# iracigt/ceres-raytracer

Measured on AMD Instinct MI355X. Metric: Mrays/sec (primary+shadow) on dragon.obj 1920x1080; 1/2/4/8-GPU scaling, higher is better.
Workload: dtype f32; 1 GPU; dragon_1080: dragon.obj 1920x1080 primary+shadow, 16 copies of the config view per step; views=config, W=1920, H=1080, row_block=1080, parallelism=one GPU, whole frames, float_framebuffer=True, streams=8

## Files before the change

### ceres-raytracer_amd/__init__.py

```python
import ctypes
import os
import sys

import numpy as np

_PKG = os.path.dirname(os.path.abspath(__file__))
LIB_PATH = os.environ.get("CERES_LIB") or os.path.join(_PKG, "libceres_hip.so")
CLI_PATH = os.path.join(_PKG, "render")

if _PKG not in sys.path:
    sys.path.insert(0, _PKG)
import configs

MODE_FULL, MODE_PRIMARY = 0, 1
MODE_ROBUST = 0x10
MODE_QBVH4 = 0x20
MODE_FMA = 0x40
ARITH_EXACT, ARITH_FMA = 0, 1


def cfg_mode(cfg, arith=ARITH_EXACT):
    return ((MODE_PRIMARY if cfg["mode"] == "primary" else MODE_FULL) | (MODE_ROBUST if cfg.get("robust") else 0)
            | (MODE_FMA if arith else 0))
SCENE_STATS = 1
# ... 5 lines not shown
    "ceres_device_free", "ceres_camera_basis", "ceres_obj_load_f64", "ceres_proc_mesh_f64", "ceres_rotate_triangles_f64",
    "ceres_bvh_build_f64", "ceres_camera_basis_f64", "ceres_orbit_cameras_f64", "ceres_scene_create_f64",
    "ceres_render_f64", "ceres_render_records_f64", "ceres_obj_load_f64_arith", "ceres_proc_mesh_f64_arith",
    "ceres_rotate_triangles_f64_arith", "ceres_bvh_build_f64_arith", "ceres_camera_basis_f64_arith",
    "ceres_orbit_cameras_f64_arith",
    "ceres_free", "ceres_scene_create", "ceres_scene_create_device", "ceres_scene_destroy", "ceres_scene_info", "ceres_scene_shadow_stacks", "ceres_render_f32",
    "ceres_render_device", "ceres_render_batch_device", "ceres_render_multi_f32", "ceres_device_count", "ceres_assemble_rgb8_packed", "ceres_render_records", "ceres_tiling_local_rows",
    "ceres_scene_set_timing", "ceres_scene_read_timing", "ceres_scene_wave_log", "ceres_fetch_counters",
    "ceres_cpu_scene_create", "ceres_cpu_scene_destroy", "ceres_render_cpu_f32", "ceres_cpu_scene_create_f64",
    "ceres_render_cpu_f64",
    "ceres_orbit_cameras", "ceres_assemble_rgb8",
    "ceres_kernel_names", "ceres_last_error", "ceres_version",
    "ceres_obj_load_arith", "ceres_proc_mesh_arith", "ceres_rotate_triangles_arith", "ceres_bvh_build_arith",
    "ceres_camera_basis_arith", "ceres_orbit_cameras_arith", "ceres_content_hash",
    "ceres_bvh_build_gpu_arith", "ceres_bvh_build_device_arith", "ceres_obj_load_gpu_arith",
    "ceres_obj_parse_device_arith", "ceres_rotate_triangles_device_arith",
)


class CeresError(RuntimeError):
    pass


class _Stats(ctypes.Structure):
    _fields_ = [("rays", ctypes.c_uint64), ("hits", ctypes.c_uint64), ("primary_rays", ctypes.c_uint64),
                ("shadow_rays", ctypes.c_uint64), ("node_pairs", ctypes.c_uint64), ("tri_tests", ctypes.c_uint64),
                ("ms", ctypes.c_double)]


class Tiling(ctypes.Structure):
    _fields_ = [("row_block", ctypes.c_uint32), ("rank", ctypes.c_uint32), ("world", ctypes.c_uint32),
# ... 112 lines not shown
    L.ceres_render_cpu_f64.argtypes = [_vp, _dp, _dp, ctypes.c_int, _dp, ctypes.POINTER(ctypes.c_uint8), _sz, _sz,
                                       ctypes.POINTER(_Stats), ctypes.c_int]
    L.ceres_content_hash.argtypes = [_vp, _sz]
    L.ceres_content_hash.restype = ctypes.c_uint64
    L.ceres_obj_load_arith.argtypes = L.ceres_obj_load.argtypes + [ctypes.c_int]
    L.ceres_proc_mesh_arith.argtypes = L.ceres_proc_mesh.argtypes + [ctypes.c_int]
    L.ceres_rotate_triangles_arith.argtypes = L.ceres_rotate_triangles.argtypes + [ctypes.c_int]
    L.ceres_bvh_build_arith.argtypes = L.ceres_bvh_build.argtypes + [ctypes.c_int]
    L.ceres_camera_basis_arith.argtypes = L.ceres_camera_basis.argtypes + [ctypes.c_int]
    L.ceres_orbit_cameras_arith.argtypes = L.ceres_orbit_cameras.argtypes + [ctypes.c_int]
    L.ceres_bvh_build_gpu_arith.argtypes = L.ceres_bvh_build_gpu.argtypes + [ctypes.c_int]
    L.ceres_bvh_build_device_arith.argtypes = L.ceres_bvh_build_device.argtypes + [ctypes.c_int]
    L.ceres_obj_load_gpu_arith.argtypes = L.ceres_obj_load_gpu.argtypes + [ctypes.c_int]
    L.ceres_obj_parse_device_arith.argtypes = L.ceres_obj_parse_device.argtypes + [ctypes.c_int]
    L.ceres_rotate_triangles_device_arith.argtypes = L.ceres_rotate_triangles_device.argtypes + [ctypes.c_int]
    _lib = L
    return L


def _check(rc):
    if rc != 0:
        raise CeresError(f"ceres error {rc}: {lib().ceres_last_error().decode()}")


def _p(a, t):
    return None if a is None else a.ctypes.data_as(ctypes.POINTER(t))


def _take(ptr, count, dtype):
    if count == 0:
# ... 127 lines not shown
    return Bvh(_take(nodes, m.value * 8, np.uint32).reshape(-1, 8), _take(prim, len(mesh), np.uint64))


def build_bvh_gpu(mesh, device=0, arith=ARITH_EXACT):
    nodes, prim, m = _u32p(), _u64p(), _sz()
    _check(lib().ceres_bvh_build_gpu_arith(_p(mesh.tri, ctypes.c_float), len(mesh), ctypes.byref(nodes),
                                           ctypes.byref(m), ctypes.byref(prim), int(device), int(arith)))
    return Bvh(_take(nodes, m.value * 8, np.uint32).reshape(-1, 8), _take(prim, len(mesh), np.uint64))


def build_bvh_device(d_tri48, n_tri, d_nodes32, d_prim32, stream=0, arith=ARITH_EXACT):
    m = _sz()
    _check(lib().ceres_bvh_build_device_arith(d_tri48, n_tri, d_nodes32, d_prim32, ctypes.byref(m), stream or None,
                                              int(arith)))
    return m.value


class CpuScene:

    def __init__(self, mesh, bvh):
        L = lib()
        self.f64 = mesh.f64
        if self.f64:
            self._h = L.ceres_cpu_scene_create_f64(_p(mesh.tri, ctypes.c_double), len(mesh), _p(mesh.norm, ctypes.c_double),
                                                   bvh.nodes.ctypes.data_as(_vp), bvh.nodes.shape[0],
                                                   _p(bvh.prim, ctypes.c_uint64))
        else:
            self._h = L.ceres_cpu_scene_create(_p(mesh.tri, ctypes.c_float), len(mesh), _p(mesh.norm, ctypes.c_float),
                                               bvh.nodes.ctypes.data_as(_vp), bvh.nodes.shape[0],
                                               _p(bvh.prim, ctypes.c_uint64))
# ... 299 lines not shown
```

### ceres-raytracer_amd/csrc/ceres_types.hpp

```cpp
#pragma once
#include <cstddef>
#include <cstdint>
#include <vector>

namespace ceres {

struct Tri48 {
    float p0[3], e1[3], e2[3], n[3];
};
static_assert(sizeof(Tri48) == 48, "Tri48");

struct RefNode {
    float bounds[6];
    uint32_t primitive_count;
    uint32_t first_child_or_primitive;
};
static_assert(sizeof(RefNode) == 32, "RefNode");

struct alignas(16) SiblingPair {
    float lb[6];
    float rb[6];
    uint32_t lcount, lfirst;
    uint32_t rcount, rfirst;
};
// ... 92 lines not shown
    uint32_t bands;
    uint32_t band_magic;
    uint32_t row_blocks_per_frame;
    uint32_t stack_entries;
    uint32_t root_leaf_count, root_leaf_first;
    float root_box[6];
    uint32_t root_box_ok;
    uint32_t cull;
    uint32_t shadow_stack_entries;
    uint32_t steal_first;
    uint32_t packets;
    uint32_t tiles_x;
    uint32_t lds_entries;
    uint32_t tile_packed;
    const uint32_t* tile_order;
    const SiblingPair* pairs;
    const Node4* nodes4;
    const QNode4* qnodes4;
    const Tri48* tris;
    const uint32_t* orig;
    const float* norms;
    float* pixels;
    uint8_t* rgb8;
    Shard* shards;
    int32_t* rec_prim;
    float* rec_tuv;
    int8_t* rec_shadow;
    unsigned long long* wave_log;
};
static_assert(sizeof(KParams) <= 4096, "KParams must fit the 4 KB kernel-argument limit");
// ... 27 lines not shown
```

### ceres-raytracer_amd/csrc/render_hip.hip

```cpp
#include <hip/hip_runtime.h>

#include <algorithm>
#include <chrono>
#include <cfloat>
#include <cmath>
#include <cstdint>
#include <cstdlib>
#include <cstring>
#include <new>
#include <string>
#include <type_traits>
#include <vector>

#include "ceres_render.h"
#include "ceres_types.hpp"
#include "host_common.hpp"
#include "pow24.hpp"

#pragma clang fp contract(off)

#ifndef CERES_COUNTING
#define CERES_COUNTING 0
#endif
#ifndef CERES_TILES_PER_WAVE
#define CERES_TILES_PER_WAVE 4
#endif
#ifndef CERES_TPW_BY_SIZE
#define CERES_TPW_BY_SIZE 1
#endif
#ifndef CERES_FRAME_MAJOR_PIXELS
#define CERES_FRAME_MAJOR_PIXELS (1u << 20)
#endif
#ifndef CERES_SPLIT_UNIFORM
#define CERES_SPLIT_UNIFORM 1
#endif
// ... 32 lines not shown
#endif
#ifndef CERES_RCP_UNIFORM
#define CERES_RCP_UNIFORM 2
#endif
#ifndef CERES_RCP_IFTHEN
#define CERES_RCP_IFTHEN 1
#endif
#ifndef CERES_PK_PACKET
#define CERES_PK_PACKET 1
#endif
#ifndef CERES_LOAD_ALWAYS
#define CERES_LOAD_ALWAYS 1
#endif
#ifndef CERES_CULL
#define CERES_CULL 1
#endif
#ifndef CERES_TRI_SELECT
#define CERES_TRI_SELECT 1
#endif

namespace ceres {

char* error_buffer() {
    static thread_local char buf[kErrorBufferSize] = "";
    return buf;
}

namespace dev {

constexpr int kBlock = 256;
// ... 239 lines not shown
        case 0: fn(std::integral_constant<int, 0>{}); break;
        case 1: fn(std::integral_constant<int, 1>{}); break;
        case 2: fn(std::integral_constant<int, 2>{}); break;
        case 3: fn(std::integral_constant<int, 3>{}); break;
        case 4: fn(std::integral_constant<int, 4>{}); break;
        case 5: fn(std::integral_constant<int, 5>{}); break;
        case 6: fn(std::integral_constant<int, 6>{}); break;
        default: fn(std::integral_constant<int, 7>{}); break;
    }
    return true;
}

template <bool kAnyHit, bool kStats, int kS = kBlock, typename StkT = uint32_t*, bool kRobust = false, int kOct = -1,
          bool kG = false>
__device__ __forceinline__ bool trace(const KParams& P, F3 o, F3 d, StkT stk, Hit& best,
                                      uint32_t& n_pairs, uint32_t& n_tests, bool& overflow) {
    const float tmin = 0.0f;
    float tmax = FLT_MAX;
    bool have = false;
    constexpr bool kU = CERES_RCP_UNIFORM == 1 || (CERES_RCP_UNIFORM == 2 && kOct == -2);
    if (P.root_leaf_count) {
        if (kStats) n_tests += P.root_leaf_count;
        for (uint32_t k = P.root_leaf_first; k < P.root_leaf_first + P.root_leaf_count; ++k) {
            float t, u, v;
            CERES_COUNT_V(kFTriV, 48);
            if (tri_test<kG, kU>(load_tri(P.tris + k), o, d, tmin, tmax, t, u, v)) {
                best = {k, t, u, v}; have = true;
                if (kAnyHit) return true;
                tmax = t;
            }
        }
        return have;
    }
    const Slab<kRobust> sl = make_slab<kRobust>(o, d);
    if constexpr (!kRobust && kOct == -1 && (CERES_OCTANT_SLAB & 1)) {
        bool r = false;
        if (with_uniform_octant(sl, [&](auto k) {
                r = trace<kAnyHit, kStats, kS, StkT, kRobust, decltype(k)::value, kG>(P, o, d, stk, best, n_pairs, n_tests, overflow);
            }))
            return r;
    }
    if (P.root_box_ok) {
        float e, x;
        slab_box<kRobust, kOct>(sl, P.root_box[0], P.root_box[1], P.root_box[2], P.root_box[3], P.root_box[4],
                          P.root_box[5], tmin, tmax, e, x);
        if (!(e <= x)) {
            if (kStats) ++n_pairs;
            return false;
        }
    }
    uint32_t sp = 0;
    if (CERES_TRI_SELECT && !kAnyHit) best.slot = kNoSlot;
    const float4* q = reinterpret_cast<const float4*>(P.pairs);
    float4 A = q[0], B = q[1], C = q[2];
    uint4 L = reinterpret_cast<const uint4*>(q)[3];
    CERES_COUNT_V(kFBvh2V, 64);
    while (true) {
        if (kStats) ++n_pairs;
        const uint32_t top = stk[(sp ? sp - 1 : 0) * kS];
        float le, lx, re, rx;
        slab_box<kRobust, kOct>(sl, A.x, A.y, A.z, A.w, B.x, B.y, tmin, tmax, le, lx);
        slab_box<kRobust, kOct>(sl, B.z, B.w, C.x, C.y, C.z, C.w, tmin, tmax, re, rx);
        const bool hit_l = le <= lx, hit_r = re <= rx;
        const bool go_l = hit_l && !L.x, go_r = hit_r && !L.z;
        const bool both = go_l && go_r, none = !go_l && !go_r;
        const bool swap = le > re;
        const bool done = none && sp == 0;
        const uint32_t near = both ? (swap ? L.w : L.y) : (go_l ? L.y : L.w);
// ... 33 lines not shown
            if (tri_test_u<kG, kU>(P.tris, idx, o, d, tmin, tmax, t, u, v)) {
                best = {idx, t, u, v}; have = true;
                if (kAnyHit) return true;
                tmax = t;
            }
        }
        if (done) break;
        A = nA; B = nB; C = nC; L = nL;
    }
    if (CERES_TRI_SELECT && !kAnyHit) return best.slot != kNoSlot;
    return have;
}

template <bool kStats, int kS, typename StkT, bool kRobust, int kOct, bool kG>
__device__ __forceinline__ bool guarded_trace(const KParams& P, F3 o, F3 d, StkT stk, Hit& best, uint32_t& n_pairs,
                                              uint32_t& n_tests, bool& overflow) {
    constexpr bool kGuard = !kStats && CERES_TRUST_STACK_BOUND && CERES_STACK_GUARD;
    const uint32_t slot = P.stack_entries * kS;
    if (kGuard) stk[slot] = stack_guard<StkT>();
    const bool hit = trace<false, kStats, kS, StkT, kRobust, kOct, kG>(P, o, d, stk, best, n_pairs, n_tests, overflow);
    if (kGuard) overflow |= uint32_t(stk[slot]) != stack_guard<StkT>();
    return hit;
}

struct N4 { float4 lx, hx, ly, hy, lz, hz; uint4 ch; };
__device__ __forceinline__ N4 load_n4(const Node4* n) {
    const float4* q = reinterpret_cast<const float4*>(n);
    const uint4* u = reinterpret_cast<const uint4*>(n);
    return {q[0], q[1], q[2], q[3], q[4], q[5], u[6]};
}
__device__ __forceinline__ uint32_t n4_count(uint32_t w) { return w & kNode4MaxCount; }
__device__ __forceinline__ uint32_t n4_first(uint32_t w) { return w >> kNode4CountBits; }
__device__ __forceinline__ N4 load_n4_u(const Node4* nodes, uint32_t cur) {
    uint32_t r;
    if (uniform_id(cur, r)) {
// ... 664 lines not shown
    bool overflow = false;
    static_assert(kTPW == 1 || kTPW == 2 || kTPW == 4 || kTPW == 8, "CERES_TILES_PER_WAVE must be 1, 2, 4 or 8");
    uint4 tiles4 = make_uint4(0, 0, 0, 0), tiles4b = make_uint4(0, 0, 0, 0);
    if constexpr (kTPW == 8) {
        tiles4 = sload_u4(P.tile_order + 8 * size_t(blockIdx.x), 0);
        tiles4b = sload_u4(P.tile_order + 8 * size_t(blockIdx.x), 1);
    } else if constexpr (kTPW == 4) {
        tiles4 = sload_u4(P.tile_order + 4 * size_t(blockIdx.x), 0);
    } else if constexpr (kTPW == 2) {
        tiles4.x = sload_u32(P.tile_order + 2 * size_t(blockIdx.x));
        tiles4.y = sload_u32(P.tile_order + 2 * size_t(blockIdx.x) + 1);
    } else {
        tiles4.x = sload_u32(P.tile_order + blockIdx.x);
    }
    CERES_COUNT_S(kFOrderS, 4 * kTPW);
    for (uint32_t q = 0; q < kTPW; ++q) {
    const uint32_t slot_q = blockIdx.x * kTPW + q;
    if (kTPW > 1 && slot_q >= n_tiles) break;
    const uint4 tq = q < 4 ? tiles4 : tiles4b;
    const uint32_t qq = q & 3;
    const uint32_t t = kTPW == 1 ? tiles4.x : qq == 0 ? tq.x : qq == 1 ? tq.y : qq == 2 ? tq.z : tq.w;
    const uint32_t qp = (q - 1) & 3;
    const uint4 tp = q - 1 < 4 ? tiles4 : tiles4b;
    const uint32_t t_prev = qp == 0 ? tp.x : qp == 1 ? tp.y : qp == 2 ? tp.z : tp.w;
    uint32_t f, lr, i;
    bool active = tile_pixel(t, f, lr, i);
    uint32_t px = (f * P.local_rows + lr) * P.W + i;
    auto redecode = [&]() {
        if constexpr (CERES_LEAN_WRITES) {
            uint32_t tr = t;
            asm volatile("" : "+s"(tr));
            active = tile_pixel(tr, f, lr, i);
            px = (f * P.local_rows + lr) * P.W + i;
        }
    };
    bool hit = false;
    Hit h{0, 0.f, 0.f, 0.f};
    RayWork w{};
    uint64_t t_start = 0;
    if (kStats && P.wave_log) t_start = __builtin_amdgcn_s_memrealtime();
    const bool last_q = q + 1 == kTPW || (kTPW > 1 && slot_q + 1 >= n_tiles);
    if (!kStats && P.cull && tile_misses_root(P, f, active, i, global_row<kBands>(P, f, lr))) {
        const float z = CERES_LEAN_WRITES ? fresh_zero() : 0.f;
        emit(q, last_q, t_prev, active, f, lr, i, z, z, z);
        continue;
    }
    if (active) {
        const F3 view = primary_dir<kG>(P, f, i, global_row<kBands>(P, f, lr));
        constexpr int kOctMode = (!kSteal || (CERES_OCTANT_SLAB & 4)) ? -1 : -2;
        hit = guarded_trace<kStats, kB, StkT, kRobust, kOctMode, kG>(P, f3(P.cam[f].eye), view, stk, h, n_pairs,
                                                                   n_tests, overflow);
        if (P.rec_prim) {
            redecode();
            P.rec_prim[px] = hit ? int32_t(P.orig[h.slot]) : -1;
            P.rec_tuv[3 * size_t(px)] = hit ? h.t : 0.f;
            P.rec_tuv[3 * size_t(px) + 1] = hit ? h.u : 0.f;
            P.rec_tuv[3 * size_t(px) + 2] = hit ? h.v : 0.f;
            P.rec_shadow[px] = -1;
        }
        if (hit) {
            CERES_COUNT_V(kFShadeV, 48);
            const TriV tr = load_tri(P.tris + h.slot);
            const F3 normal = normalizeG<kG>(tr.n);
            w = make_shadow_ray<kRobust, kG>(hit_point<kG>(tr, normal, h.u, h.v), f3(P.cam[f].sun));
        }
    }
// ... 31 lines not shown
    const uint32_t shard = blockIdx.x % kShards;
    if (lane == 0 && n_shadow) {
        atomicAdd(&P.shards[shard].queued, n_shadow);
        atomicAdd(&P.shards[shard].hits, (unsigned long long)(n_shadow + wo));
    }
    if (kStats) {
        const uint32_t wp = wave_sum(n_pairs), wt = wave_sum(n_tests);
        if (lane == 0) {
            atomicAdd(&P.shards[shard].pairs, (unsigned long long)wp);
            atomicAdd(&P.shards[shard].tests, (unsigned long long)wt);
        }
    }
    if (overflow) atomicOr(&P.shards[shard].error, 1u);
}

__global__ __launch_bounds__(256) void ceres_compact_lit(const float* __restrict__ px, uint32_t n_pix,
                                                         uint4* __restrict__ out, uint32_t* __restrict__ n,
                                                         uint32_t cap) {
    const uint32_t p = blockIdx.x * 256 + threadIdx.x, lane = threadIdx.x & 63;
    uint32_t r = 0, g = 0, b = 0;
    if (p < n_pix) {
        const float* q = px + 3 * size_t(p);
        r = __float_as_uint(q[0]); g = __float_as_uint(q[1]); b = __float_as_uint(q[2]);
    }
    const bool lit = (r | g | b) != 0;
    const uint64_t m = __ballot(lit);
    if (!m) return;
    uint32_t base = 0;
    if (lane == 0) base = atomicAdd(n, uint32_t(__popcll(m)));
    base = uint32_t(__shfl(int(base), 0, 64));
// ... 64 lines not shown
    do {                                                                                      \
        hipError_t e_ = (expr);                                                               \
        if (e_ != hipSuccess) return set_error(CERES_EHIP, "%s: %s", #expr, hipGetErrorString(e_)); \
    } while (0)

template <typename T>
void dfree(T*& p) { if (p) { (void)hipFree(p); p = nullptr; } }

}

void ceres::scene_release(ceres_scene* s) {
    if (!s) return;
    (void)hipSetDevice(s->device);
    dfree(s->d_pairs64); dfree(s->d_tris64); dfree(s->d_norms64);
    for (auto& o : s->orders) dfree(o.d);
    for (auto& d : s->retired) dfree(d);
    s->orders.clear(); s->retired.clear(); s->retired_bytes = 0;
    dfree(s->d_pairs); dfree(s->d_nodes4); dfree(s->d_qnodes4); dfree(s->d_tris); dfree(s->d_orig); dfree(s->d_norms);
    dfree(s->d_shards); dfree(s->d_counters); dfree(s->d_wave_log); dfree(s->d_pixels); dfree(s->d_rgb8);
    for (auto e : s->ev_pool) (void)hipEventDestroy(e);
    for (auto e : s->ev_used) (void)hipEventDestroy(e);
    s->ev_pool.clear(); s->ev_used.clear();
    for (auto e : s->band_events) (void)hipEventDestroy(e);
    s->band_events.clear();
    dfree(s->d_band_counters);
    dfree(s->d_lit); dfree(s->d_lit_count);
    if (s->h_lit_pinned) (void)hipHostFree(s->h_lit_pinned);
    s->h_lit_pinned = nullptr;
    if (s->h_small) (void)hipHostFree(s->h_small);
    s->h_small = nullptr;
// ... 259 lines not shown
        const double pw = r[0] * c0[0] + r[1] * c0[1] + r[2] * c0[2], qw = r[0] * c1[0] + r[1] * c1[1] + r[2] * c1[2];
        const double ww = r[0] * c2[0] + r[1] * c2[1] + r[2] * c2[2];
        if (!(ww / det > 0.01 * std::sqrt(r[0] * r[0] + r[1] * r[1] + r[2] * r[2]))) return keep;
        u0 = std::min(u0, pw / ww); u1 = std::max(u1, pw / ww); v0 = std::min(v0, qw / ww); v1 = std::max(v1, qw / ww);
    }
    const double m = 2e-3 * (1 + std::max(std::max(std::fabs(u0), std::fabs(u1)), std::max(std::fabs(v0), std::fabs(v1))));
    auto lo = [](double x, uint32_t n) { return x <= 0 ? 0u : x >= n ? n : uint32_t(std::floor(x)); };
    const double a0 = (u0 - m + 1) * W / 2 - 0.5 - 1, a1 = (u1 + m + 1) * W / 2 - 0.5 + 1;
    const double b0 = (v0 - m + 1) * H / 2 - 0.5 - 1, b1 = (v1 + m + 1) * H / 2 - 0.5 + 1;
    if (!(a0 == a0 && a1 == a1 && b0 == b0 && b1 == b1)) return keep;
    if (a1 < 0 || b1 < 0) return CullRect{1u, 0u, 1u, 0u};
    return CullRect{uint16_t(lo(a0, W)), uint16_t(std::min<double>(std::ceil(a1), 0xffff)),
                    uint16_t(lo(b0, H)), uint16_t(std::min<double>(std::ceil(b1), 0xffff))};
}

static int stack_width(size_t n_pairs, size_t n_nodes4) {
    const size_t nmax = std::max(n_pairs, n_nodes4);
    return CERES_STACK16 && nmax < (1u << 16) ? 2 : CERES_STACK24 && nmax < (1u << 24) ? 3 : 4;
}
static uint32_t batch_tiles_per_wave(size_t frame_pixels, int stw, bool qbvh) {
    if (!CERES_TPW_BY_SIZE || stw != 2 || qbvh) return CERES_TILES_PER_WAVE;
    return frame_pixels >= (size_t(1) << 20) && frame_pixels < (size_t(1) << 22) ? 2u : uint32_t(CERES_TILES_PER_WAVE);
}

static size_t fused_lds_bytes(uint32_t entries, int stw) {
    return size_t(entries) * dev::kFusedB * stw + sizeof(dev::StealLdsT<dev::kFusedB>);
}
static bool lds_limits_waves(uint32_t entries, int stw) { return fused_lds_bytes(entries, stw) > dev::kLdsPerCu / 28; }

static int check_fused_lds(const ceres_scene* s, const KParams& P, int stw, size_t dyn_bytes) {
    const size_t need = size_t(P.lds_entries) * dev::kFusedB * size_t(stw);
    const size_t total = dyn_bytes + sizeof(dev::StealLdsT<dev::kFusedB>);
    if (stw != 2 && stw != 3 && stw != 4)
        return set_error(CERES_EINVAL, "render: bad LDS stack entry width %d", stw);
    if (P.lds_entries < P.stack_entries + 1 || P.lds_entries < P.shadow_stack_entries || dyn_bytes < need)
        return set_error(CERES_EINVAL, "render: LDS stack of %u slots (%zu B) cannot hold the BVH2 stack (%u + 1) and the BVH4 "
                         "stack (%u)", P.lds_entries, dyn_bytes, P.stack_entries, P.shadow_stack_entries);
    if (total > s->max_lds_per_block)
        return set_error(CERES_EINVAL, "render: fused kernel needs %zu B of LDS per workgroup (%zu available)", total,
                         s->max_lds_per_block);
    return CERES_OK;
}

int launch_chunk(ceres_scene* s, uint32_t frames, const float* basis12, const float* sun, int mode, size_t W, size_t H,
                 const ceres_tiling* tiling, float* d_pixels, uint8_t* d_rgb8, uint64_t* d_counters, hipStream_t stream,
                 int32_t* d_rec_prim, float* d_rec_tuv, int8_t* d_rec_shadow, bool first, bool last,
                 uint64_t batch_primary) {
// ... 77 lines not shown
    const bool need_clean = d_counters || !full;
    if (first && need_clean && s->shards_dirty) HIP_TRY(hipMemsetAsync(s->d_shards, 0, sizeof(Shard) * kShards, stream));
    s->shards_dirty = true;
    if (rows) {
        if (e0) HIP_TRY(hipEventRecord(e0, stream));
        if (full) {
            const int stw = stack_width(s->n_pairs, s->n_nodes4);
            const bool st16 = stw == 2;
            const bool steal = frames == 1 && !t.bands;
            P.steal_first = steal && !stats && ((s->flags & CERES_SCENE_FIRST_ORDER) ||
                                                lds_limits_waves(std::max(s->stack_entries + 1, s->shadow_stack_entries), stw))
                                ? 1u : 0u;
            P.shadow_stack_entries = (!steal || P.steal_first) ? s->shadow_stack_first : s->shadow_stack_entries;
            P.lds_entries = uint32_t(std::max(s->stack_entries + 1, P.shadow_stack_entries));
            const size_t flds = size_t(P.lds_entries) * dev::kFusedB * stw;
            if (int rc = check_fused_lds(s, P, stw, flds)) return rc;
            if (!stats)
                if (const char* g = std::getenv("CERES_DEBUG_GUARD_SLOT")) {
                    const long k = std::strtol(g, nullptr, 10);
                    if (k > 0 && uint32_t(k) < P.stack_entries) P.stack_entries = uint32_t(k);
                }
            P.tile_order = tile_order;
            P.tile_packed = packed ? 1u : 0u;
            P.tiles_x = fbx;
            P.row_blocks_per_frame = fby;
            const uint32_t n_tiles = fbx * fby * frames;
            const dim3 fgrid((n_tiles + tpw - 1) / tpw), fblock(dev::kFusedB);
            if (stats) {
                const size_t waves = size_t(fbx) * fby * frames;
                if (s->wave_log_waves < waves) {
                    dfree(s->d_wave_log);
                    HIP_TRY(hipMalloc(&s->d_wave_log, waves * 64));
                    s->wave_log_waves = waves;
                }
                HIP_TRY(hipMemsetAsync(s->d_wave_log, 0, waves * 64, stream));
                P.wave_log = s->d_wave_log;
                s->last_grid_waves = waves;
            }
            constexpr int w32 = CERES_FUSED_MINW32;
            auto fused = [&](auto rt, auto st, auto gt) {
                constexpr bool R = decltype(rt)::value, T = decltype(st)::value, G = decltype(gt)::value;
                constexpr int w16 = T ? CERES_FUSED_MINW16_SOLO : CERES_FUSED_MINW16;
// ... 124 lines not shown

extern "C" {

const char* ceres_last_error(void) { return error_buffer(); }
extern const char ceres_src_sha[];
const char* ceres_version(void) {
    static const std::string v = std::string("ceres-mi355x 0.3 (gfx950) src ") + ceres_src_sha;
    return v.c_str();
}
int ceres_device_count(void) {
    int n = 0;
    if (hipGetDeviceCount(&n) != hipSuccess) return set_error(CERES_EHIP, "hipGetDeviceCount failed");
    return n;
}
const char* ceres_kernel_names(void) {
    return "ceres_fused,ceres_primary,ceres_finalize,ceres_assemble";
}

size_t ceres_tiling_local_rows(size_t height, const ceres_tiling* t) {
    if (!t) return height;
    if (t->world == 0 || t->row_block == 0 || t->rank >= t->world) return 0;
    return local_rows_of(height, *t);
}

ceres_scene* ceres_scene_create(const float* tri48, size_t n_tri, const float* norm36, const void* nodes32,
                                size_t n_nodes, const uint64_t* prim64, int device, uint32_t flags) {
    if (!tri48 || !norm36 || !nodes32 || !prim64 || n_tri == 0 || n_nodes == 0) {
        set_error(CERES_EINVAL, "ceres_scene_create: empty scene or null argument");
        return nullptr;
    }
    if (n_tri > 0xffffffffull || n_nodes > 0xffffffffull) { set_error(CERES_EUNSUPPORTED, "scene too large"); return nullptr; }
// ... 521 lines not shown
```

### ceres-raytracer_amd/csrc/scene_internal.hpp

```cpp
#pragma once
#include <hip/hip_runtime.h>

#include <cstdint>
#include <utility>
#include <vector>

#include "ceres_types.hpp"

using ceres::SiblingPair; using ceres::SiblingPair64; using ceres::Node4; using ceres::Tri48; using ceres::Tri96;
using ceres::Shard;

struct ceres_scene {
    int device = 0;
    uint32_t flags = 0;
    size_t n_tri = 0, n_pairs = 0;
    uint32_t depth = 0, stack_entries = 1, root_leaf_count = 0, root_leaf_first = 0;
    float root_box[6] = {0, 0, 0, 0, 0, 0};
    uint32_t root_box_ok = 0;
    uint32_t shadow_stack_entries = 1;
    uint32_t shadow_stack_first = 1;
    size_t n_nodes4 = 0;
    SiblingPair* d_pairs = nullptr;
    Node4* d_nodes4 = nullptr;
    ceres::QNode4* d_qnodes4 = nullptr;
    struct TileOrder {
        size_t W = 0, H = 0;
        uint32_t row_block = 0, rank = 0, world = 0, frames = 0, tile = 0, bands = 0;
        bool packed = false;
        uint32_t* d = nullptr;
        size_t cap = 0;
        uint64_t used = 0;
    };
    std::vector<TileOrder> orders;
    std::vector<uint32_t*> retired;
    size_t retired_bytes = 0;
    uint64_t order_clock = 0;
    Tri48* d_tris = nullptr;
    uint32_t* d_orig = nullptr;
    float* d_norms = nullptr;
    Shard* d_shards = nullptr;
    bool shards_dirty = true;
    uint64_t* d_counters = nullptr;
    float* d_pixels = nullptr;
    uint8_t* d_rgb8 = nullptr;
    size_t px_cap = 0;
    hipStream_t stream = nullptr;
    hipStream_t copy_stream = nullptr;
    uint64_t* d_band_counters = nullptr;
// ... 39 lines not shown
```

### include/ceres_render.h

```cpp
#ifndef CERES_RENDER_H
#define CERES_RENDER_H

#include <stddef.h>
#include <stdint.h>

#ifdef __cplusplus
extern "C" {
#endif

typedef enum {
    CERES_OK = 0,
    CERES_EINVAL = -1,
    CERES_EIO = -2,
    CERES_ENOMEM = -3,
    CERES_EHIP = -4,
    CERES_ESTACK = -5,
    CERES_EUNSUPPORTED = -6
} ceres_status;

typedef enum {
    CERES_MODE_FULL = 0,
    CERES_MODE_PRIMARY = 1,
    CERES_MODE_ROBUST = 0x10,
    CERES_MODE_QBVH4 = 0x20,
// ... 133 lines not shown
int ceres_fetch_counters(int device, uint64_t out[8], int reset);

typedef struct ceres_cpu_scene ceres_cpu_scene;
ceres_cpu_scene* ceres_cpu_scene_create(const float* tri48, size_t n_tri, const float* norm36, const void* nodes32,
                                        size_t n_nodes, const uint64_t* prim64);
void ceres_cpu_scene_destroy(ceres_cpu_scene* scene);
int ceres_render_cpu_f32(const ceres_cpu_scene* scene, const float basis12[12], const float sun[3], int mode,
                         float* pixels, uint8_t* rgb8, size_t width, size_t height, ceres_stats* stats, int threads);
ceres_cpu_scene* ceres_cpu_scene_create_f64(const double* tri96, size_t n_tri, const double* norm72, const void* nodes64,
                                            size_t n_nodes, const uint64_t* prim64);
int ceres_render_cpu_f64(const ceres_cpu_scene* scene, const double basis12[12], const double sun[3], int mode,
                         double* pixels, uint8_t* rgb8, size_t width, size_t height, ceres_stats* stats, int threads);

uint64_t ceres_content_hash(const void* p, size_t bytes);

const char* ceres_kernel_names(void);

const char* ceres_last_error(void);
const char* ceres_version(void);

#ifdef __cplusplus
}
#endif

#endif
```

Baseline: 47910 Mrays/s.

## Precompute per-tile BVH entry nodes to start primary traversal below the root

Adds a small pre-pass kernel that, for each 8x8 pixel tile, walks down the BVH in double precision while only one child's box can project into the tile's padded frustum, and records that node (or a miss marker). The fused render kernel then loads this per-tile entry and starts primary traversal from it, and uses the miss marker in place of the existing root-cull test. This is meant to skip the top-level node visits that every primary ray in a tile would repeat. In exchange it adds an extra kernel launch and a per-stream device buffer. It is only enabled for full non-robust, non-stealing renders with culling on, and a host-side reference function is added for testing.

```diff
diff --git a/ceres-raytracer_amd/__init__.py b/ceres-raytracer_amd/__init__.py
--- a/ceres-raytracer_amd/__init__.py
+++ b/ceres-raytracer_amd/__init__.py
@@ -43,7 +43,7 @@
     "ceres_obj_load_arith", "ceres_proc_mesh_arith", "ceres_rotate_triangles_arith", "ceres_bvh_build_arith",
     "ceres_camera_basis_arith", "ceres_orbit_cameras_arith", "ceres_content_hash",
     "ceres_bvh_build_gpu_arith", "ceres_bvh_build_device_arith", "ceres_obj_load_gpu_arith",
-    "ceres_obj_parse_device_arith", "ceres_rotate_triangles_device_arith",
+    "ceres_obj_parse_device_arith", "ceres_rotate_triangles_device_arith", "ceres_tile_entries_host",
 )
 
 
@@ -186,6 +186,10 @@
     L.ceres_obj_load_gpu_arith.argtypes = L.ceres_obj_load_gpu.argtypes + [ctypes.c_int]
     L.ceres_obj_parse_device_arith.argtypes = L.ceres_obj_parse_device.argtypes + [ctypes.c_int]
     L.ceres_rotate_triangles_device_arith.argtypes = L.ceres_rotate_triangles_device.argtypes + [ctypes.c_int]
+    if hasattr(L, "ceres_tile_entries_host"):
+        L.ceres_tile_entries_host.argtypes = [_fp, _sz, _vp, _sz, _u64p, ctypes.c_uint32, _fp, _sz, _sz, ctypes.POINTER(Tiling),
+                                              _u32p, _u32p, ctypes.POINTER(_u32p), ctypes.POINTER(_sz),
+                                              ctypes.POINTER(_u32p)]
     _lib = L
     return L
 
@@ -343,6 +347,25 @@
     _check(lib().ceres_bvh_build_device_arith(d_tri48, n_tri, d_nodes32, d_prim32, ctypes.byref(m), stream or None,
                                               int(arith)))
     return m.value
+
+
+def tile_entries_host(mesh, bvh, basis12, W, H, tiling=None, want_layout=False):
+    b = np.ascontiguousarray(basis12, np.float32).reshape(-1, 12)
+    t = tiling if tiling is not None else Tiling(H, 0, 1, 0)
+    rows = lib().ceres_tiling_local_rows(H, ctypes.byref(t))
+    fby, fbx = (rows + 7) // 8, (W + 7) // 8
+    out = np.zeros((b.shape[0], fby, fbx), np.uint32)
+    steps = np.zeros((b.shape[0], fby, fbx), np.uint32)
+    pp, n, oo = _u32p(), _sz(), _u32p()
+    _check(lib().ceres_tile_entries_host(_p(mesh.tri, ctypes.c_float), len(mesh), bvh.nodes.ctypes.data_as(_vp),
+                                         bvh.nodes.shape[0], _p(bvh.prim, ctypes.c_uint64), b.shape[0],
+                                         _p(b, ctypes.c_float), W, H, ctypes.byref(t), _p(out, ctypes.c_uint32),
+                                         _p(steps, ctypes.c_uint32),
+                                         ctypes.byref(pp) if want_layout else None, ctypes.byref(n),
+                                         ctypes.byref(oo) if want_layout else None))
+    if not want_layout:
+        return out
+    return out, steps, _take(pp, max(1, n.value) * 16, np.uint32).reshape(-1, 16)[:n.value], _take(oo, len(mesh), np.uint32)
 
 
 class CpuScene:
diff --git a/ceres-raytracer_amd/csrc/ceres_types.hpp b/ceres-raytracer_amd/csrc/ceres_types.hpp
--- a/ceres-raytracer_amd/csrc/ceres_types.hpp
+++ b/ceres-raytracer_amd/csrc/ceres_types.hpp
@@ -130,6 +130,7 @@
     uint32_t lds_entries;
     uint32_t tile_packed;
     const uint32_t* tile_order;
+    const uint32_t* entry;
     const SiblingPair* pairs;
     const Node4* nodes4;
     const QNode4* qnodes4;
diff --git a/ceres-raytracer_amd/csrc/render_hip.hip b/ceres-raytracer_amd/csrc/render_hip.hip
--- a/ceres-raytracer_amd/csrc/render_hip.hip
+++ b/ceres-raytracer_amd/csrc/render_hip.hip
@@ -19,6 +19,8 @@
 
 #pragma clang fp contract(off)
 
+#include "tile_entry.hpp"
+
 #ifndef CERES_COUNTING
 #define CERES_COUNTING 0
 #endif
@@ -81,6 +83,12 @@
 #endif
 #ifndef CERES_CULL
 #define CERES_CULL 1
+#endif
+#ifndef CERES_TILE_ENTRY
+#define CERES_TILE_ENTRY 1
+#endif
+#ifndef CERES_TILE_ENTRY_SOLO
+#define CERES_TILE_ENTRY_SOLO 0
 #endif
 #ifndef CERES_TRI_SELECT
 #define CERES_TRI_SELECT 1
@@ -350,7 +358,7 @@
 template <bool kAnyHit, bool kStats, int kS = kBlock, typename StkT = uint32_t*, bool kRobust = false, int kOct = -1,
           bool kG = false>
 __device__ __forceinline__ bool trace(const KParams& P, F3 o, F3 d, StkT stk, Hit& best,
-                                      uint32_t& n_pairs, uint32_t& n_tests, bool& overflow) {
+                                      uint32_t& n_pairs, uint32_t& n_tests, bool& overflow, uint32_t entry = 0u) {
     const float tmin = 0.0f;
     float tmax = FLT_MAX;
     bool have = false;
@@ -372,7 +380,7 @@
     if constexpr (!kRobust && kOct == -1 && (CERES_OCTANT_SLAB & 1)) {
         bool r = false;
         if (with_uniform_octant(sl, [&](auto k) {
-                r = trace<kAnyHit, kStats, kS, StkT, kRobust, decltype(k)::value, kG>(P, o, d, stk, best, n_pairs, n_tests, overflow);
+                r = trace<kAnyHit, kStats, kS, StkT, kRobust, decltype(k)::value, kG>(P, o, d, stk, best, n_pairs, n_tests, overflow, entry);
             }))
             return r;
     }
@@ -387,7 +395,7 @@
     }
     uint32_t sp = 0;
     if (CERES_TRI_SELECT && !kAnyHit) best.slot = kNoSlot;
-    const float4* q = reinterpret_cast<const float4*>(P.pairs);
+    const float4* q = reinterpret_cast<const float4*>(P.pairs + entry);
     float4 A = q[0], B = q[1], C = q[2];
     uint4 L = reinterpret_cast<const uint4*>(q)[3];
     CERES_COUNT_V(kFBvh2V, 64);
@@ -451,11 +459,11 @@
 
 template <bool kStats, int kS, typename StkT, bool kRobust, int kOct, bool kG>
 __device__ __forceinline__ bool guarded_trace(const KParams& P, F3 o, F3 d, StkT stk, Hit& best, uint32_t& n_pairs,
-                                              uint32_t& n_tests, bool& overflow) {
+                                              uint32_t& n_tests, bool& overflow, uint32_t entry = 0u) {
     constexpr bool kGuard = !kStats && CERES_TRUST_STACK_BOUND && CERES_STACK_GUARD;
     const uint32_t slot = P.stack_entries * kS;
     if (kGuard) stk[slot] = stack_guard<StkT>();
-    const bool hit = trace<false, kStats, kS, StkT, kRobust, kOct, kG>(P, o, d, stk, best, n_pairs, n_tests, overflow);
+    const bool hit = trace<false, kStats, kS, StkT, kRobust, kOct, kG>(P, o, d, stk, best, n_pairs, n_tests, overflow, entry);
     if (kGuard) overflow |= uint32_t(stk[slot]) != stack_guard<StkT>();
     return hit;
 }
@@ -1150,12 +1158,30 @@
         tiles4.x = sload_u32(P.tile_order + blockIdx.x);
     }
     CERES_COUNT_S(kFOrderS, 4 * kTPW);
+    constexpr bool kEntry = !kStats && !kRobust;
+    uint4 ent4 = make_uint4(0, 0, 0, 0), ent4b = make_uint4(0, 0, 0, 0);
+    if (kEntry && P.entry) {
+        auto ld = [&](uint32_t t_) {
+            uint32_t id = t_;
+            if (P.tile_packed)
+                id = ((t_ >> (kTileXBits + kTileYBits)) * P.row_blocks_per_frame + ((t_ >> kTileXBits) & ((1u << kTileYBits) - 1u))) *
+                         P.tiles_x + (t_ & ((1u << kTileXBits) - 1u));
+            return sload_u32(P.entry + id);
+        };
+        ent4.x = ld(tiles4.x);
+        if constexpr (kTPW >= 2) ent4.y = ld(tiles4.y);
+        if constexpr (kTPW >= 4) { ent4.z = ld(tiles4.z); ent4.w = ld(tiles4.w); }
+        if constexpr (kTPW == 8) { ent4b.x = ld(tiles4b.x); ent4b.y = ld(tiles4b.y); ent4b.z = ld(tiles4b.z); ent4b.w = ld(tiles4b.w); }
+        CERES_COUNT_S(kFOrderS, 4 * kTPW);
+    }
     for (uint32_t q = 0; q < kTPW; ++q) {
     const uint32_t slot_q = blockIdx.x * kTPW + q;
     if (kTPW > 1 && slot_q >= n_tiles) break;
     const uint4 tq = q < 4 ? tiles4 : tiles4b;
     const uint32_t qq = q & 3;
     const uint32_t t = kTPW == 1 ? tiles4.x : qq == 0 ? tq.x : qq == 1 ? tq.y : qq == 2 ? tq.z : tq.w;
+    const uint4 eq = q < 4 ? ent4 : ent4b;
+    const uint32_t ent = !kEntry ? 0u : kTPW == 1 ? ent4.x : qq == 0 ? eq.x : qq == 1 ? eq.y : qq == 2 ? eq.z : eq.w;
     const uint32_t qp = (q - 1) & 3;
     const uint4 tp = q - 1 < 4 ? tiles4 : tiles4b;
     const uint32_t t_prev = qp == 0 ? tp.x : qp == 1 ? tp.y : qp == 2 ? tp.z : tp.w;
@@ -1176,7 +1202,7 @@
     uint64_t t_start = 0;
     if (kStats && P.wave_log) t_start = __builtin_amdgcn_s_memrealtime();
     const bool last_q = q + 1 == kTPW || (kTPW > 1 && slot_q + 1 >= n_tiles);
-    if (!kStats && P.cull && tile_misses_root(P, f, active, i, global_row<kBands>(P, f, lr))) {
+    if (!kStats && ((kEntry && P.entry) ? ent == kEntryMiss : (P.cull && tile_misses_root(P, f, active, i, global_row<kBands>(P, f, lr))))) {
         const float z = CERES_LEAN_WRITES ? fresh_zero() : 0.f;
         emit(q, last_q, t_prev, active, f, lr, i, z, z, z);
         continue;
@@ -1185,7 +1211,7 @@
         const F3 view = primary_dir<kG>(P, f, i, global_row<kBands>(P, f, lr));
         constexpr int kOctMode = (!kSteal || (CERES_OCTANT_SLAB & 4)) ? -1 : -2;
         hit = guarded_trace<kStats, kB, StkT, kRobust, kOctMode, kG>(P, f3(P.cam[f].eye), view, stk, h, n_pairs,
-                                                                   n_tests, overflow);
+                                                                   n_tests, overflow, ent);
         if (P.rec_prim) {
             redecode();
             P.rec_prim[px] = hit ? int32_t(P.orig[h.slot]) : -1;
@@ -1247,6 +1273,23 @@
     if (overflow) atomicOr(&P.shards[shard].error, 1u);
 }
 
+template <bool kBands>
+__global__ __launch_bounds__(256) void ceres_entries(const KParams P, uint32_t* __restrict__ out) {
+    const uint32_t per_frame = P.tiles_x * P.row_blocks_per_frame;
+    const uint32_t id = blockIdx.x * 256 + threadIdx.x, f = blockIdx.y;
+    if (id >= per_frame) return;
+    const uint32_t by = id / P.tiles_x, bx = id - by * P.tiles_x;
+    const uint32_t i0 = bx * 8u, i1 = min(i0 + 7u, P.W - 1u);
+    const uint32_t lr0 = by * 8u, lr1 = min(lr0 + 7u, P.local_rows - 1u);
+    const uint32_t j0 = tiling_global_row(P.row_block, P.rank, P.world, kBands ? 1u : 0u, f, lr0);
+    const uint32_t j1 = tiling_global_row(P.row_block, P.rank, P.world, kBands ? 1u : 0u, f, lr1);
+    const CullRect r = P.cull_rect[f];
+    uint32_t e = kEntryMiss;
+    if (!(i1 < r.i0 || i0 > r.i1 || j1 < r.j0 || j0 > r.j1))
+        e = tile_entry(entry_frame(P.cam[f], P.root_box), entry_range(i0, i1, j0, j1, P.W, P.H), P.pairs);
+    out[size_t(f) * per_frame + id] = e;
+}
+
 __global__ __launch_bounds__(256) void ceres_compact_lit(const float* __restrict__ px, uint32_t n_pix,
                                                          uint4* __restrict__ out, uint32_t* __restrict__ n,
                                                          uint32_t cap) {
@@ -1341,6 +1384,8 @@
     (void)hipSetDevice(s->device);
     dfree(s->d_pairs64); dfree(s->d_tris64); dfree(s->d_norms64);
     for (auto& o : s->orders) dfree(o.d);
+    for (auto& b : s->entry_bufs) dfree(b.d);
+    s->entry_bufs.clear();
     for (auto& d : s->retired) dfree(d);
     s->orders.clear(); s->retired.clear(); s->retired_bytes = 0;
     dfree(s->d_pairs); dfree(s->d_nodes4); dfree(s->d_qnodes4); dfree(s->d_tris); dfree(s->d_orig); dfree(s->d_norms);
@@ -1630,6 +1675,37 @@
                     uint16_t(lo(b0, H)), uint16_t(std::min<double>(std::ceil(b1), 0xffff))};
 }
 
+constexpr size_t kMaxEntryBufs = 32;
+int ensure_entry_buf(ceres_scene* s, hipStream_t stream, size_t n, uint32_t** out) {
+    ceres_scene::EntryBuf* b = nullptr;
+    for (auto& e : s->entry_bufs)
+        if (e.stream == stream) { b = &e; break; }
+    if (!b) {
+        if (s->entry_bufs.size() >= kMaxEntryBufs) {
+            auto lru = std::min_element(s->entry_bufs.begin(), s->entry_bufs.end(),
+                                        [](const auto& x, const auto& y) { return x.used < y.used; });
+            dfree(lru->d);
+            s->entry_bufs.erase(lru);
+        }
+        s->entry_bufs.push_back(ceres_scene::EntryBuf{stream, nullptr, 0, 0});
+        b = &s->entry_bufs.back();
+    }
+    if (b->cap < n) {
+        dfree(b->d);
+        b->cap = 0;
+        const size_t cap = (n + 1023) / 1024 * 1024;
+        HIP_TRY(hipMalloc(&b->d, cap * sizeof(uint32_t)));
+        b->cap = cap;
+    }
+    b->used = ++s->order_clock;
+    *out = b->d;
+    return CERES_OK;
+}
+
+static bool use_tile_entry(const KParams& P, bool full, bool steal, bool robust) {
+    return CERES_TILE_ENTRY && (CERES_TILE_ENTRY_SOLO || !steal) && full && !robust && P.cull && !P.root_leaf_count;
+}
+
 static int stack_width(size_t n_pairs, size_t n_nodes4) {
     const size_t nmax = std::max(n_pairs, n_nodes4);
     return CERES_STACK16 && nmax < (1u << 16) ? 2 : CERES_STACK24 && nmax < (1u << 24) ? 3 : 4;
@@ -1644,9 +1720,9 @@
 }
 static bool lds_limits_waves(uint32_t entries, int stw) { return fused_lds_bytes(entries, stw) > dev::kLdsPerCu / 28; }
 
-static int check_fused_lds(const ceres_scene* s, const KParams& P, int stw, size_t dyn_bytes) {
+static int check_fused_lds(const ceres_scene* s, const KParams& P, int stw, size_t dyn_bytes, bool pair_stash) {
     const size_t need = size_t(P.lds_entries) * dev::kFusedB * size_t(stw);
-    const size_t total = dyn_bytes + sizeof(dev::StealLdsT<dev::kFusedB>);
+    const size_t total = dyn_bytes + sizeof(dev::StealLdsT<dev::kFusedB>) + (pair_stash ? sizeof(dev::PairStash) : 0);
     if (stw != 2 && stw != 3 && stw != 4)
         return set_error(CERES_EINVAL, "render: bad LDS stack entry width %d", stw);
     if (P.lds_entries < P.stack_entries + 1 || P.lds_entries < P.shadow_stack_entries || dyn_bytes < need)
@@ -1754,18 +1830,29 @@
             P.shadow_stack_entries = (!steal || P.steal_first) ? s->shadow_stack_first : s->shadow_stack_entries;
             P.lds_entries = uint32_t(std::max(s->stack_entries + 1, P.shadow_stack_entries));
             const size_t flds = size_t(P.lds_entries) * dev::kFusedB * stw;
-            if (int rc = check_fused_lds(s, P, stw, flds)) return rc;
+            if (int rc = check_fused_lds(s, P, stw, flds, CERES_PAIR_STORES && !stats && !steal && tpw >= 2 && st16)) return rc;
+#if CERES_STACK_GUARD
             if (!stats)
                 if (const char* g = std::getenv("CERES_DEBUG_GUARD_SLOT")) {
                     const long k = std::strtol(g, nullptr, 10);
                     if (k > 0 && uint32_t(k) < P.stack_entries) P.stack_entries = uint32_t(k);
                 }
+#endif
             P.tile_order = tile_order;
             P.tile_packed = packed ? 1u : 0u;
             P.tiles_x = fbx;
             P.row_blocks_per_frame = fby;
             const uint32_t n_tiles = fbx * fby * frames;
             const dim3 fgrid((n_tiles + tpw - 1) / tpw), fblock(dev::kFusedB);
+            if (use_tile_entry(P, full, steal, robust)) {
+                uint32_t* d_entry = nullptr;
+                if (int rc = ensure_entry_buf(s, stream, n_tiles, &d_entry)) return rc;
+                P.entry = d_entry;
+                const dim3 egrid((fbx * fby + 255) / 256, frames), eblock(256);
+                if (t.bands) hipLaunchKernelGGL(dev::ceres_entries<true>, egrid, eblock, 0, stream, P, d_entry);
+                else hipLaunchKernelGGL(dev::ceres_entries<false>, egrid, eblock, 0, stream, P, d_entry);
+                HIP_TRY(hipGetLastError());
+            }
             if (stats) {
                 const size_t waves = size_t(fbx) * fby * frames;
                 if (s->wave_log_waves < waves) {
@@ -1920,7 +2007,63 @@
     return n;
 }
 const char* ceres_kernel_names(void) {
-    return "ceres_fused,ceres_primary,ceres_finalize,ceres_assemble";
+    return "ceres_fused,ceres_primary,ceres_entries,ceres_finalize,ceres_assemble";
+}
+
+int ceres_tile_entries_host(const float* tri48, size_t n_tri, const void* nodes32, size_t n_nodes, const uint64_t* prim64,
+                            uint32_t frames, const float* basis12, size_t width, size_t height, const ceres_tiling* tiling,
+                            uint32_t* entries, uint32_t* steps, uint32_t** pairs16, size_t* n_pairs, uint32_t** orig) {
+    if (!tri48 || !nodes32 || !prim64 || !basis12 || !entries || n_tri == 0 || n_nodes == 0 || width == 0 || height == 0)
+        return set_error(CERES_EINVAL, "ceres_tile_entries_host: null or empty argument");
+    ceres_tiling t{uint32_t(height), 0, 1};
+    if (tiling) t = *tiling;
+    if (t.world == 0 || t.rank >= t.world || t.row_block == 0) return set_error(CERES_EINVAL, "ceres_tile_entries_host: bad tiling");
+    if (t.world == 1) t.bands = 0;
+    std::vector<SiblingPair> pairs;
+    std::vector<Tri48> leaf_tris;
+    std::vector<uint32_t> og;
+    uint32_t depth = 0, rlc = 0, rlf = 0;
+    if (int rc = relayout_bvh(static_cast<const RefNode*>(nodes32), n_nodes, prim64, n_tri, reinterpret_cast<const Tri48*>(tri48),
+                              pairs, leaf_tris, og, depth, rlc, rlf))
+        return rc;
+    const float* root = static_cast<const RefNode*>(nodes32)[0].bounds;
+    const bool ok = !rlc && !pairs.empty() && box_inside(pairs[0].lb, root) && box_inside(pairs[0].rb, root);
+    const size_t rows = local_rows_of(height, t);
+    const uint32_t fbx = uint32_t((width + 7) / 8), fby = uint32_t((rows + 7) / 8);
+    for (uint32_t f = 0; f < frames; ++f) {
+        FrameCam c{};
+        std::memcpy(c.eye, basis12 + 12 * f, 12); std::memcpy(c.dir, basis12 + 12 * f + 3, 12);
+        std::memcpy(c.iu, basis12 + 12 * f + 6, 12); std::memcpy(c.iv, basis12 + 12 * f + 9, 12);
+        const CullRect r = cull_rect(c, root, uint32_t(width), uint32_t(height));
+        const EntryFrame F = entry_frame(c, root);
+        for (uint32_t by = 0; by < fby; ++by)
+            for (uint32_t bx = 0; bx < fbx; ++bx) {
+                const uint32_t i0 = bx * 8u, i1 = std::min<uint32_t>(i0 + 7u, uint32_t(width) - 1u);
+                const uint32_t lr0 = by * 8u, lr1 = std::min<uint32_t>(lr0 + 7u, uint32_t(rows) - 1u);
+                const uint32_t j0 = tiling_global_row(t.row_block, t.rank, t.world, t.bands, f, lr0);
+                const uint32_t j1 = tiling_global_row(t.row_block, t.rank, t.world, t.bands, f, lr1);
+                uint32_t e = 0, n = 0;
+                if (ok && CERES_TILE_ENTRY && CERES_CULL && CERES_ROOT_TEST) {
+                    e = kEntryMiss;
+                    if (!(i1 < r.i0 || i0 > r.i1 || j1 < r.j0 || j0 > r.j1))
+                        e = tile_entry(F, entry_range(i0, i1, j0, j1, uint32_t(width), uint32_t(height)), pairs.data(), &n);
+                }
+                entries[(size_t(f) * fby + by) * fbx + bx] = e;
+                if (steps) steps[(size_t(f) * fby + by) * fbx + bx] = n;
+            }
+    }
+    if (pairs16) {
+        *pairs16 = static_cast<uint32_t*>(std::malloc(std::max<size_t>(1, pairs.size()) * sizeof(SiblingPair)));
+        if (!*pairs16) return set_error(CERES_ENOMEM, "out of host memory");
+        std::memcpy(*pairs16, pairs.data(), pairs.size() * sizeof(SiblingPair));
+    }
+    if (n_pairs) *n_pairs = pairs.size();
+    if (orig) {
+        *orig = static_cast<uint32_t*>(std::malloc(std::max<size_t>(1, og.size()) * sizeof(uint32_t)));
+        if (!*orig) return set_error(CERES_ENOMEM, "out of host memory");
+        std::memcpy(*orig, og.data(), og.size() * sizeof(uint32_t));
+    }
+    return CERES_OK;
 }
 
 size_t ceres_tiling_local_rows(size_t height, const ceres_tiling* t) {
diff --git a/ceres-raytracer_amd/csrc/scene_internal.hpp b/ceres-raytracer_amd/csrc/scene_internal.hpp
--- a/ceres-raytracer_amd/csrc/scene_internal.hpp
+++ b/ceres-raytracer_amd/csrc/scene_internal.hpp
@@ -32,6 +32,13 @@
         uint64_t used = 0;
     };
     std::vector<TileOrder> orders;
+    struct EntryBuf {
+        hipStream_t stream = nullptr;
+        uint32_t* d = nullptr;
+        size_t cap = 0;
+        uint64_t used = 0;
+    };
+    std::vector<EntryBuf> entry_bufs;
     std::vector<uint32_t*> retired;
     size_t retired_bytes = 0;
     uint64_t order_clock = 0;
diff --git a/ceres-raytracer_amd/csrc/tile_entry.hpp b/ceres-raytracer_amd/csrc/tile_entry.hpp
--- /dev/null
+++ b/ceres-raytracer_amd/csrc/tile_entry.hpp
@@ -0,0 +1,103 @@
+#pragma once
+#include <cstdint>
+
+#include "ceres_types.hpp"
+
+#if defined(__HIPCC__)
+#define CERES_TE_HD __host__ __device__
+#else
+#define CERES_TE_HD
+#endif
+
+namespace ceres {
+
+constexpr uint32_t kEntryMiss = 0xffffffffu;
+constexpr uint32_t kEntryMaxSteps = 96;
+
+struct EntryFrame {
+    double c[3][3];
+    double e[3];
+    double pad;
+    bool ok;
+};
+
+CERES_TE_HD inline EntryFrame entry_frame(const FrameCam& cam, const float root[6]) {
+    EntryFrame F;
+    double iu[3], iv[3], d[3];
+    for (int k = 0; k < 3; ++k) { F.e[k] = cam.eye[k]; iu[k] = cam.iu[k]; iv[k] = cam.iv[k]; d[k] = cam.dir[k]; }
+    double sc = 0;
+    for (int k = 0; k < 3; ++k) { const double a = F.e[k] < 0 ? -F.e[k] : F.e[k]; sc = a > sc ? a : sc; }
+    for (int k = 0; k < 6; ++k) { const double r = root[k]; const double a = r < 0 ? -r : r; sc = a > sc ? a : sc; }
+    F.pad = 1e-4 * sc;
+    F.c[0][0] = iv[1] * d[2] - iv[2] * d[1]; F.c[0][1] = iv[2] * d[0] - iv[0] * d[2]; F.c[0][2] = iv[0] * d[1] - iv[1] * d[0];
+    F.c[1][0] = d[1] * iu[2] - d[2] * iu[1]; F.c[1][1] = d[2] * iu[0] - d[0] * iu[2]; F.c[1][2] = d[0] * iu[1] - d[1] * iu[0];
+    F.c[2][0] = iu[1] * iv[2] - iu[2] * iv[1]; F.c[2][1] = iu[2] * iv[0] - iu[0] * iv[2]; F.c[2][2] = iu[0] * iv[1] - iu[1] * iv[0];
+    const double det = iu[0] * F.c[0][0] + iu[1] * F.c[0][1] + iu[2] * F.c[0][2];
+    const double inv = 1.0 / det;
+    F.ok = det != 0 && inv == inv && inv - inv == 0 && sc - sc == 0;
+    for (int r = 0; r < 3; ++r)
+        for (int k = 0; k < 3; ++k) F.c[r][k] *= inv;
+    return F;
+}
+
+struct EntryRange { double ulo, uhi, vlo, vhi; };
+CERES_TE_HD inline EntryRange entry_range(uint32_t i0, uint32_t i1, uint32_t j0, uint32_t j1, uint32_t W, uint32_t H) {
+    EntryRange R;
+    R.ulo = 2 * (double(i0) - 0.5) / double(W) - 1; R.uhi = 2 * (double(i1) + 1.5) / double(W) - 1;
+    R.vlo = 2 * (double(j0) - 0.5) / double(H) - 1; R.vhi = 2 * (double(j1) + 1.5) / double(H) - 1;
+    auto ab = [](double x) { return x < 0 ? -x : x; };
+    double mx = ab(R.ulo);
+    mx = ab(R.uhi) > mx ? ab(R.uhi) : mx; mx = ab(R.vlo) > mx ? ab(R.vlo) : mx; mx = ab(R.vhi) > mx ? ab(R.vhi) : mx;
+    const double m = 2e-3 * (1 + mx);
+    R.ulo -= m; R.uhi += m; R.vlo -= m; R.vhi += m;
+    return R;
+}
+
+CERES_TE_HD inline bool box_invisible(const EntryFrame& F, const EntryRange& R, const float b[6]) {
+    bool gt_u = true, lt_u = true, gt_v = true, lt_v = true;
+    for (int k = 0; k < 8; ++k) {
+        const double r0 = ((k & 1) ? double(b[1]) + F.pad : double(b[0]) - F.pad) - F.e[0];
+        const double r1 = ((k & 2) ? double(b[3]) + F.pad : double(b[2]) - F.pad) - F.e[1];
+        const double r2 = ((k & 4) ? double(b[5]) + F.pad : double(b[4]) - F.pad) - F.e[2];
+        const double p = r0 * F.c[0][0] + r1 * F.c[0][1] + r2 * F.c[0][2];
+        const double q = r0 * F.c[1][0] + r1 * F.c[1][1] + r2 * F.c[1][2];
+        const double w = r0 * F.c[2][0] + r1 * F.c[2][1] + r2 * F.c[2][2];
+        if (!(w > 0 && w * w > 1e-4 * (r0 * r0 + r1 * r1 + r2 * r2))) return false;
+        gt_u = gt_u && p - R.uhi * w > 0; lt_u = lt_u && p - R.ulo * w < 0;
+        gt_v = gt_v && q - R.vhi * w > 0; lt_v = lt_v && q - R.vlo * w < 0;
+    }
+    return gt_u || lt_u || gt_v || lt_v;
+}
+
+CERES_TE_HD inline bool box_inside(const float c[6], const float o[6]) {
+    return c[0] >= o[0] && c[1] <= o[1] && c[2] >= o[2] && c[3] <= o[3] && c[4] >= o[4] && c[5] <= o[5];
+}
+
+CERES_TE_HD inline uint32_t tile_entry(const EntryFrame& F, const EntryRange& R, const SiblingPair* pairs,
+                                       uint32_t* n_steps = nullptr) {
+    if (!F.ok) return 0u;
+    uint32_t cur = 0;
+    for (uint32_t step = 0; step < kEntryMaxSteps; ++step) {
+        if (n_steps) ++*n_steps;
+        const SiblingPair& p = pairs[cur];
+        const bool vl = !box_invisible(F, R, p.lb), vr = !box_invisible(F, R, p.rb);
+        if (!vl && !vr) return kEntryMiss;
+        if (vl && vr) return cur;
+        const uint32_t count = vl ? p.lcount : p.rcount, first = vl ? p.lfirst : p.rfirst;
+        if (count) return cur;
+        const float* cb = vl ? p.lb : p.rb;
+        const SiblingPair& n = pairs[first];
+        if (!box_inside(n.lb, cb) || !box_inside(n.rb, cb)) return cur;
+        cur = first;
+    }
+    return cur;
+}
+
+CERES_TE_HD inline uint32_t tiling_global_row(uint32_t row_block, uint32_t rank, uint32_t world, uint32_t bands, uint32_t f,
+                                           uint32_t lr) {
+    if (world == 1) return lr;
+    if (bands) return ((rank + f) % world) * row_block + lr;
+    return ((lr / row_block) * world + rank) * row_block + lr % row_block;
+}
+
+}
diff --git a/include/ceres_render.h b/include/ceres_render.h
--- a/include/ceres_render.h
+++ b/include/ceres_render.h
@@ -171,6 +171,11 @@
 
 uint64_t ceres_content_hash(const void* p, size_t bytes);
 
+int ceres_tile_entries_host(const float* tri48, size_t n_tri, const void* nodes32, size_t n_nodes,
+                            const uint64_t* prim64, uint32_t frames, const float* basis12, size_t width,
+                            size_t height, const ceres_tiling* tiling, uint32_t* entries, uint32_t* steps,
+                            uint32_t** pairs16, size_t* n_pairs, uint32_t** orig);
+
 const char* ceres_kernel_names(void);
 
 const char* ceres_last_error(void);
```

Result: slower. 44110 Mrays/s (-7.9%).
